# PinataFarms/DAD-3DHeads

Measured on AMD Instinct MI355X. Metric: images/sec (FLAME decode + 445-lmk projection), batch 64 @ 256^2, higher is better.
Workload: dtype f32

## Files before the change

dad-3dheads_amd/csrc/flame_decode_head.hip:

```cpp
#pragma clang fp contract(off)
#include "common.hpp"
#include "flame_math.hpp"
#include "flame_pipe_epilogue.hpp"

#ifndef DAD3D_HEAD_DEPTH
#define DAD3D_HEAD_DEPTH 6
#endif
#ifndef DAD3D_HEAD_R0_AT
#define DAD3D_HEAD_R0_AT 1
#endif

namespace dad3d {

namespace {

using namespace pipe;

constexpr int KG = kPipeKGroups;
constexpr int TV = kPipeTileVerts;
constexpr int kNumBeta = 400;
constexpr int kJawCol = 3 * TV;
constexpr int LD = 424;
constexpr int OS = 76;
constexpr int CS = 24;
constexpr int kRows = 64;
constexpr int kRows1 = 48;
constexpr int kRound = 128;
constexpr int D = DAD3D_HEAD_DEPTH < KG ? DAD3D_HEAD_DEPTH : KG;
static_assert(D >= 6 && DAD3D_HEAD_R0_AT < D, "issue-ahead depth");
struct Lds {
    static constexpr int a_off = 0;
    static constexpr int o_off = a_off + kRows * LD;
    static constexpr int c_off = o_off + kRows * OS;
    static constexpr int y_off = c_off + 2 * kRound * CS;
    static constexpr int v_off = y_off + 4;
    static constexpr int total = v_off + 4 * TV;
    static_assert(total * 4 <= 160 * 1024, "LDS budget of one CU");
};

__device__ __forceinline__ int lds_peek(lds_int* p) { return __hip_atomic_load(p, __ATOMIC_RELAXED, __HIP_MEMORY_SCOPE_WORKGROUP); }
__device__ __forceinline__ void wait_ge(lds_int* p, int target) {
    while (lds_peek(p) < target) __builtin_amdgcn_s_sleep(1);
    asm volatile("" ::: "memory");
}
__device__ __forceinline__ void wait_ge2(lds_int* p, int target, lds_int* q, int target_q) {
    while ((int)(lds_peek(p) < target) | (int)(lds_peek(q) < target_q)) __builtin_amdgcn_s_sleep(1);
    asm volatile("" ::: "memory");
}
__device__ __forceinline__ void arrive(lds_int* p, int lane) {
    asm volatile("s_waitcnt lgkmcnt(0)" ::: "memory");
    if (lane == 0) __hip_atomic_fetch_add(p, 1, __ATOMIC_RELAXED, __HIP_MEMORY_SCOPE_WORKGROUP);
}
__device__ __forceinline__ void phase_barrier() {
    asm volatile("s_waitcnt lgkmcnt(0)\n\ts_barrier" ::: "memory");
}

}

constexpr int kHeadPreloadDwords = 14;
static_assert(4 * kHeadPreloadDwords == 4 * sizeof(void*) + 6 * sizeof(int), "the preloaded range ends with n_lmk");
struct PipeLateArgs {
    const int* lmk_next;
    float *verts3d, *proj, *lmk_xy;
    int32_t* lmk_px;
    float image_size;
};
static_assert((4 * kHeadPreloadDwords) % alignof(PipeLateArgs) == 0, "`late` starts where the preloaded range ends: late_args() reads it there");
template <bool TO2D>
__global__ __launch_bounds__(512, 2) void flame_decode_head_kernel(float* params, const float* bpack, const float4* vtab, unsigned long long* trace_buf, int batch,
                                                                   int n_verts, int n_params, int span_half, unsigned geom, int n_lmk, PipeLateArgs late) {
    PipeArgs a;
    a.params = params, a.bpack = bpack, a.vtab = vtab, a.trace = trace_buf, a.n_params = n_params, a.batch = batch, a.n_half = span_half, a.n_verts = n_verts, a.n_lmk = n_lmk;
    a.flags = pipe_geom_unpack(geom).flags;
    extern __shared__ __attribute__((aligned(16))) float smem[];
    float* abuf = smem + Lds::a_off;
    float* otile = smem + Lds::o_off;
    float* cst = smem + Lds::c_off;
    lds_int* parts = (lds_int*)(smem + Lds::y_off);

    const int tid = threadIdx.x, lane = tid & 63, wave = tid >> 6;
    const int tile = blockIdx.x, v0 = tile * TV;
    const int B = a.batch, P = a.n_params;
    const bool two = B > kRows1;
    unsigned long long* trace = a.trace ? a.trace + ((size_t)tile * 8 + wave) * 32 : nullptr;
    auto stamp = [&](int slot) {
        if (trace && lane == 0) trace[slot] = __builtin_readcyclecounter();
    };
    if (trace && lane == 0) trace[12] = wall_clock64();
    stamp(0);
    if (tid < 4) __hip_atomic_store(parts + tid, 0, __ATOMIC_RELAXED, __HIP_MEMORY_SCOPE_WORKGROUP);
    const unsigned nl = (unsigned)a.n_lmk;
    EpiCtx cx;
    __amdgpu_buffer_rsrc_t rs3, rsp;
    unsigned outs = 0;
    auto late_args = [&]() {
        typedef const __attribute__((address_space(4))) char* kernarg_ptr;
        typedef const __attribute__((address_space(4))) PipeLateArgs* late_ptr;
        kernarg_ptr kp = (kernarg_ptr)__builtin_amdgcn_kernarg_segment_ptr();
        asm volatile("" : "+s"(kp));
        const late_ptr lp = reinterpret_cast<late_ptr>(kp + 4 * kHeadPreloadDwords);
        a.lmk_next = lp->lmk_next, a.verts3d = lp->verts3d, a.proj = lp->proj, a.lmk_xy = lp->lmk_xy, a.lmk_px = lp->lmk_px, a.image_size = lp->image_size;
        rs3 = __builtin_amdgcn_make_buffer_rsrc(reinterpret_cast<char*>(a.verts3d), 0, 0x7fffffff, 0x00020000);
        rsp = __builtin_amdgcn_make_buffer_rsrc(reinterpret_cast<char*>(a.proj), 0, 0x7fffffff, 0x00020000);
        cx.lx = reinterpret_cast<char*>(a.lmk_xy), cx.lp = reinterpret_cast<char*>(a.lmk_px);
        outs = __builtin_amdgcn_readfirstlane((a.verts3d ? 1u : 0u) | (a.proj ? 2u : 0u));
        asm volatile("" : "+s"(outs));
        cx.lmk_next = a.lmk_next;
        cx.image_size = a.image_size;
    };
    cx.zsign = (a.flags & DAD3D_FLIP_Z) ? -1.0f : 1.0f;
    float4* const vt_lds = reinterpret_cast<float4*>(smem + Lds::v_off);
    auto fin4 = [&](int row0, int w) {
        const int fi = lane & 3, fu = lane >> 2, b = row0 + 4 * w + fi;
        const float4* cp = reinterpret_cast<const float4*>(cst + b * CS);
        const float4 c0 = cp[0], c1 = cp[1], c2 = cp[2], c3 = cp[3], c4 = cp[4], c5 = cp[5];
        const float* ot = otile + b * OS;
        const float jx = ot[kJawCol], jy = ot[kJawCol + 1], jz = ot[kJawCol + 2];
        const unsigned vrow = (unsigned)b * (unsigned)a.n_verts + (unsigned)(v0 + fu), bnl = (unsigned)b * nl;
        {
            const float4 t = vt_lds[fu];
            const bool live = b < B && v0 + fu < a.n_verts;
            finish_vertex<TO2D, 0>(cx, rs3, rsp, c0, c1, c2, c3, c4, c5, jx, jy, jz, ot[3 * fu], ot[3 * fu + 1], ot[3 * fu + 2], t.x, t.y, __float_as_int(t.z), __float_as_int(t.w),
                                   live && (outs & 1u), live && (outs & 2u), live && nl > 0 && __float_as_int(t.z) >= 0, vrow, bnl);
        }
        if (fu < TV - 16) {
            const int j = fu + 16;
            const float4 t = vt_lds[j];
            const bool live = b < B && v0 + j < a.n_verts;
            finish_vertex<TO2D, 16>(cx, rs3, rsp, c0, c1, c2, c3, c4, c5, jx, jy, jz, ot[3 * j], ot[3 * j + 1], ot[3 * j + 2], t.x, t.y, __float_as_int(t.z), __float_as_int(t.w),
                                    live && (outs & 1u), live && (outs & 2u), live && nl > 0 && __float_as_int(t.z) >= 0, vrow, bnl);
        }
    };
    auto fin2 = [&](int row0) {
        const int fi = lane & 1, fu = min(lane >> 1, TV - 1), b = row0 + 2 * wave + fi;
        const float4* cp = reinterpret_cast<const float4*>(cst + b * CS);
        const float4 c0 = cp[0], c1 = cp[1], c2 = cp[2], c3 = cp[3], c4 = cp[4], c5 = cp[5];
        const float* ot = otile + b * OS;
        const float jx = ot[kJawCol], jy = ot[kJawCol + 1], jz = ot[kJawCol + 2];
        const unsigned vrow = (unsigned)b * (unsigned)a.n_verts + (unsigned)(v0 + fu), bnl = (unsigned)b * nl;
        const float4 t = vt_lds[fu];
        const bool live = b < B && (lane >> 1) < TV && v0 + fu < a.n_verts;
        finish_vertex<TO2D, 0>(cx, rs3, rsp, c0, c1, c2, c3, c4, c5, jx, jy, jz, ot[3 * fu], ot[3 * fu + 1], ot[3 * fu + 2], t.x, t.y, __float_as_int(t.z), __float_as_int(t.w),
                               live && (outs & 1u), live && (outs & 2u), live && nl > 0 && __float_as_int(t.z) >= 0, vrow, bnl);
    };

    if (wave >= 4) {
        const int fw = wave - 4;
        const int lr = lane >> 5, lc = lane & 31;
        float4 pre[19];
        const float* prow[6];
#pragma unroll
        for (int jj = 0; jj < 6; ++jj) prow[jj] = a.params + (size_t)min(12 * fw + 2 * jj + lr, B - 1) * P + 4 * lc;
        auto load_slab = [&](int sl) {
#pragma unroll
            for (int jj = 0; jj < 6; ++jj) {
                const f4u v = *reinterpret_cast<const f4u*>(prow[jj] + 128 * sl);
                pre[6 * sl + jj] = float4{v.x, v.y, v.z, v.w};
                __builtin_amdgcn_sched_barrier(0);
            }
        };
        auto write_slab = [&](int sl) {
#pragma unroll
            for (int jj = 0; jj < 6; ++jj) *reinterpret_cast<float4*>(abuf + (12 * fw + 2 * jj + lr) * LD + 128 * sl + 4 * lc) = pre[6 * sl + jj];
        };
        load_slab(0);
        const float4 vt_row = a.vtab[min(v0 + min(lane, TV - 1), a.n_verts - 1)];
        stamp(1);
        phase_barrier();
        stamp(6);
        load_slab(1);
        load_slab(2);
        {
            const int r = min(lane >> 2, 11);
            const f4u v = *reinterpret_cast<const f4u*>(a.params + (size_t)min(12 * fw + r, B - 1) * P + 384 + 4 * (lane & 3));
            pre[18] = float4{v.x, v.y, v.z, v.w};
        }
        late_args();
        write_slab(0);
        arrive(parts, lane);
        stamp(7);
        write_slab(1);
        arrive(parts + 1, lane);
        write_slab(2);
        if (lane < 48) *reinterpret_cast<float4*>(abuf + (12 * fw + (lane >> 2)) * LD + 384 + 4 * (lane & 3)) = pre[18];
        arrive(parts + 2, lane);
        if (fw == 3 && lane < TV) vt_lds[lane] = vt_row;
        stamp(2);
        if (two) {
            float4 q[7];
            const float* qrow[2];
#pragma unroll
            for (int jj = 0; jj < 2; ++jj) qrow[jj] = a.params + (size_t)min(kRows1 + 4 * fw + 2 * jj + lr, B - 1) * P + 4 * lc;
#pragma unroll
            for (int sl = 0; sl < 3; ++sl)
#pragma unroll
                for (int jj = 0; jj < 2; ++jj) {
                    const f4u v = *reinterpret_cast<const f4u*>(qrow[jj] + 128 * sl);
                    q[2 * sl + jj] = float4{v.x, v.y, v.z, v.w};
                }
            {
                const f4u v = *reinterpret_cast<const f4u*>(a.params + (size_t)min(kRows1 + 4 * fw + min(lane >> 2, 3), B - 1) * P + 384 + 4 * (lane & 3));
                q[6] = float4{v.x, v.y, v.z, v.w};
            }
            stamp(16);
#pragma unroll
            for (int sl = 0; sl < 3; ++sl)
#pragma unroll
                for (int jj = 0; jj < 2; ++jj) *reinterpret_cast<float4*>(abuf + (kRows1 + 4 * fw + 2 * jj + lr) * LD + 128 * sl + 4 * lc) = q[2 * sl + jj];
            if (lane < 16) *reinterpret_cast<float4*>(abuf + (kRows1 + 4 * fw + (lane >> 2)) * LD + 384 + 4 * (lane & 3)) = q[6];
            stamp(17);
        }
        stamp(18);
        phase_barrier();
        stamp(19);
        if (two) {
            fin4(32, fw);
            stamp(21);
            phase_barrier();
            stamp(23);
            fin2(kRows1);
        } else {
            fin4(0, wave);
            fin2(32);
        }
        stamp(5);
        if (trace && lane == 0) trace[13] = wall_clock64();
        return;
    }

    const float4* bsrc = reinterpret_cast<const float4*>(a.bpack) + ((size_t)tile * KG * 4 + wave) * 64 + lane;
    f4u raw0 = {}, raw1 = {};
    f3u raw2 = {};
    float raw_scale = 0.f;
    {
        const float* prow = a.params + (size_t)min(32 * wave + (lane & 31), B - 1) * P + kNumBeta;
        raw0 = *reinterpret_cast<const f4u*>(prow), raw1 = *reinterpret_cast<const f4u*>(prow + 4), raw2 = *reinterpret_cast<const f3u*>(prow + 8);
        raw_scale = prow[12];
    }
    auto write_round = [&]() {
        const float jaw[3] = {raw0.x, raw0.y, raw0.z};
        const float rot6[6] = {raw0.w, raw1.x, raw1.y, raw1.z, raw1.w, raw2.x};
        float Dm[9], G[9];
        rodrigues_minus_identity_lean(jaw, Dm);
        rot6_to_matrix_lean(rot6, G);
        const float sp1 = raw_scale + 1.0f;
        const float s = sp1 < 1e-8f ? 1e-8f : sp1;
        if (wave < 2 && lane < 32) {
            float4* tail = reinterpret_cast<float4*>(abuf + (32 * wave + lane) * LD + kNumBeta);
            tail[0] = float4{Dm[0], Dm[1], Dm[2], Dm[3]};
            tail[1] = float4{Dm[4], Dm[5], Dm[6], Dm[7]};
            tail[2] = float4{Dm[8], 1.0f, 0.f, 0.f};
            tail[3] = float4{0.f, 0.f, 0.f, 0.f};
        }
        if (lane < 32) {
            float4* c = reinterpret_cast<float4*>(cst + (32 * wave + lane) * CS);
            c[0] = float4{Dm[0], Dm[1], Dm[2], Dm[3]};
            c[1] = float4{Dm[4], Dm[5], Dm[6], Dm[7]};
            c[2] = float4{Dm[8], G[0], G[1], G[2]};
            c[3] = float4{G[3], G[4], G[5], G[6]};
            c[4] = float4{G[7], G[8], s, raw2.y};
            c[5] = float4{raw2.z, 0.f, 0.f, 0.f};
            const int b = 32 * wave + lane;
            if ((a.flags & DAD3D_MUTATE_PARAMS) && tile == 0 && b < B)
                store_tz(a.params + ((unsigned)b * (unsigned)P + (unsigned)(kNumBeta + 11)));
        }
    };
    float4 bq[KG];
    const float* afrag0 = abuf + (lane & 15) * LD + 4 * (lane >> 4);
    float* const ot0 = otile + ((lane >> 4) * 4) * OS + wave * 16 + (lane & 15);

    late_args();
    stamp(6);
    phase_barrier();
    stamp(7);
#pragma unroll
    for (int G = 0; G < D; ++G) {
        bq[G] = bsrc[(size_t)G * 256];
        __builtin_amdgcn_sched_barrier(0);
        if (G == DAD3D_HEAD_R0_AT) {
            write_round();
            if (wave < 2) arrive(parts + 2, lane);
            arrive(parts + 3, lane);
            stamp(4);
            __builtin_amdgcn_sched_barrier(0);
        }
    }
    {
        f32x4 acc[3] = {f32x4{0.f, 0.f, 0.f, 0.f}, f32x4{0.f, 0.f, 0.f, 0.f}, f32x4{0.f, 0.f, 0.f, 0.f}};
        float4 af[3], an[3] = {};
        stamp(16);
        wait_ge(parts, 4);
#pragma unroll
        for (int m = 0; m < 3; ++m) af[m] = *reinterpret_cast<const float4*>(afrag0 + m * 16 * LD);
#pragma unroll
        for (int G = 0; G < KG; ++G) {
            if (G + D < KG) bq[G + D] = bsrc[(size_t)(G + D) * 256];
            if (G + 1 == 8) wait_ge(parts + 1, 4);
            if (G + 1 == 16) wait_ge2(parts + 2, 6, parts + 3, 4);
            if (G + 1 < KG) {
#pragma unroll
                for (int m = 0; m < 3; ++m) an[m] = *reinterpret_cast<const float4*>(afrag0 + m * 16 * LD + 16 * (G + 1));
            }
            __builtin_amdgcn_sched_barrier(0);
            if (G == 0) stamp(8);
#pragma unroll
            for (int s = 0; s < 4; ++s) {
                const float bv = s == 0 ? bq[G].x : s == 1 ? bq[G].y : s == 2 ? bq[G].z : bq[G].w;
#pragma unroll
                for (int m = 0; m < 3; ++m) {
                    const float av = s == 0 ? af[m].x : s == 1 ? af[m].y : s == 2 ? af[m].z : af[m].w;
                    acc[m] = __builtin_amdgcn_mfma_f32_16x16x4f32(av, bv, acc[m], 0, 0, 0);
                }
            }
            __builtin_amdgcn_sched_barrier(0);
#pragma unroll
            for (int m = 0; m < 3; ++m) af[m] = an[m];
        }
        stamp(2);
#pragma unroll
        for (int m = 0; m < 3; ++m)
#pragma unroll
            for (int q = 0; q < 4; ++q) ot0[(m * 16 + q) * OS] = acc[m][q];
        stamp(17);
    }
    if (!two) {
        phase_barrier();
        stamp(18);
        stamp(3);
        fin4(0, wave);
        fin2(32);
        stamp(5);
        if (trace && lane == 0) trace[13] = wall_clock64();
        return;
    }
    const int ei = lane & 7, eu = lane >> 3, li = 8 * wave + ei;
    float4 k0, k1, k2, k3, k4, k5;
    {
        const float4* c = reinterpret_cast<const float4*>(cst + li * CS);
        k0 = c[0], k1 = c[1], k2 = c[2], k3 = c[3], k4 = c[4], k5 = c[5];
    }
    phase_barrier();
    stamp(18);
    float vW[3], vw2[3];
    int lh[3], ln[3];
    bool vl[3];
#pragma unroll
    for (int k = 0; k < 3; ++k) {
        const float4 t = vt_lds[min(eu + 8 * k, TV - 1)];
        vW[k] = t.x, vw2[k] = t.y, lh[k] = __float_as_int(t.z), ln[k] = __float_as_int(t.w);
        vl[k] = eu + 8 * k < TV && v0 + eu + 8 * k < a.n_verts;
    }
    float jx = 0.f, jy = 0.f, jz = 0.f, ex = 0.f, ey = 0.f, ez = 0.f;
    const float* const ot_e = otile + li * OS;
    const unsigned e_vrow = (unsigned)li * (unsigned)a.n_verts + (unsigned)(v0 + eu), e_bnl = (unsigned)li * nl;
    bool live3[3], livep[3], livel[3];
#pragma unroll
    for (int k = 0; k < 3; ++k) live3[k] = vl[k] && (outs & 1u), livep[k] = vl[k] && (outs & 2u), livel[k] = vl[k] && nl > 0 && lh[k] >= 0;
    auto epi_fetch = [&](int k) {
        const int j = eu + 8 * k;
        ex = ot_e[3 * j], ey = ot_e[3 * j + 1], ez = ot_e[3 * j + 2];
    };
    auto epi_finish = [&](int k) {
        if (k == 0) finish_vertex<TO2D, 0>(cx, rs3, rsp, k0, k1, k2, k3, k4, k5, jx, jy, jz, ex, ey, ez, vW[0], vw2[0], lh[0], ln[0], live3[0], livep[0], livel[0], e_vrow, e_bnl);
        if (k == 1) finish_vertex<TO2D, 8>(cx, rs3, rsp, k0, k1, k2, k3, k4, k5, jx, jy, jz, ex, ey, ez, vW[1], vw2[1], lh[1], ln[1], live3[1], livep[1], livel[1], e_vrow, e_bnl);
        if (k == 2) finish_vertex<TO2D, 16>(cx, rs3, rsp, k0, k1, k2, k3, k4, k5, jx, jy, jz, ex, ey, ez, vW[2], vw2[2], lh[2], ln[2], live3[2], livep[2], livel[2], e_vrow, e_bnl);
    };
    {
        f32x4 acc = f32x4{0.f, 0.f, 0.f, 0.f};
        const float* afrag = afrag0 + kRows1 * LD;
        float4 af = *reinterpret_cast<const float4*>(afrag), an = {};
        stamp(20);
#pragma unroll
        for (int G = 0; G < KG; ++G) {
            if (G + 1 < KG) an = *reinterpret_cast<const float4*>(afrag + 16 * (G + 1));
            __builtin_amdgcn_sched_barrier(0);
            acc = __builtin_amdgcn_mfma_f32_16x16x4f32(af.x, bq[G].x, acc, 0, 0, 0);
            acc = __builtin_amdgcn_mfma_f32_16x16x4f32(af.y, bq[G].y, acc, 0, 0, 0);
            acc = __builtin_amdgcn_mfma_f32_16x16x4f32(af.z, bq[G].z, acc, 0, 0, 0);
            acc = __builtin_amdgcn_mfma_f32_16x16x4f32(af.w, bq[G].w, acc, 0, 0, 0);
            __builtin_amdgcn_sched_barrier(0);
            af = an;
            if (G == 0) {
                jx = ot_e[kJawCol], jy = ot_e[kJawCol + 1], jz = ot_e[kJawCol + 2];
                epi_fetch(0);
            }
            if (G == 3) epi_finish(0), epi_fetch(1);
            if (G == 11) epi_finish(1), epi_fetch(2);
            if (G == 19) epi_finish(2);
            __builtin_amdgcn_sched_barrier(0);
        }
#pragma unroll
        for (int q = 0; q < 4; ++q) ot0[(kRows1 + q) * OS] = acc[q];
        stamp(21);
    }
    phase_barrier();
    stamp(22);
    stamp(3);
    fin2(kRows1);
    stamp(5);
    if (trace && lane == 0) trace[13] = wall_clock64();
}

dad3d_status launch_flame_decode_head(const PipeArgs& a, hipStream_t s) {
    static PerDeviceOnce attr_done;
    const int dev = PerDeviceOnce::current();
    const size_t lds = (size_t)Lds::total * sizeof(float);
    DAD3D_REQUIRE(a.batch > kPipeHalf && a.batch <= kRows && a.chunk_half == 0 && (a.verts3d || a.proj),
                  "launch_flame_decode_head: a whole-mesh launch of 33..64 rows with a vertex output, not %d rows", a.batch);
    if (!attr_done.done(dev)) {
        for (const void* k : {reinterpret_cast<const void*>(&flame_decode_head_kernel<true>), reinterpret_cast<const void*>(&flame_decode_head_kernel<false>)})
            DAD3D_HIP_TRY(hipFuncSetAttribute(k, hipFuncAttributeMaxDynamicSharedMemorySize, (int)lds));
        attr_done.set(dev);
    }
    const bool to2d = (a.flags & DAD3D_TO_2D) || !a.proj;
    const unsigned geom = pipe_geom_word(a.flags, 0, 1, 0);
    const PipeLateArgs late{a.lmk_next, a.verts3d, a.proj, a.lmk_xy, a.lmk_px, a.image_size};
    if (to2d)
        hipLaunchKernelGGL((flame_decode_head_kernel<true>), dim3(a.n_tiles), dim3(512), lds, s, a.params, a.bpack, a.vtab, a.trace, a.batch, a.n_verts, a.n_params, a.n_half, geom,
                           a.n_lmk, late);
    else
        hipLaunchKernelGGL((flame_decode_head_kernel<false>), dim3(a.n_tiles), dim3(512), lds, s, a.params, a.bpack, a.vtab, a.trace, a.batch, a.n_verts, a.n_params, a.n_half, geom,
                           a.n_lmk, late);
    DAD3D_HIP_TRY(hipGetLastError());
    return DAD3D_OK;
}

}
```

Measured before the change: 5.769 million.

## Interleave B-fragment requests and LDS loads among MFMAs; move v16 epilogue to stagers

The global B-fragment prefetch is moved to the middle of each k-step, after the second MFMA row. The next A-fragment LDS reads are issued one per MFMA, spread through the first row, so memory instructions interleave with matrix ops instead of clustering before them. Separately, the epilogue work for vertices 16+ in the 48-row tile leaves the MFMA waves and goes to the staging waves through a new fin_v16 pass, which lightens the compute loop. The risks are more sched_barrier constraints, register pressure, and a possible imbalance between wave groups before the phase barrier.

```diff
diff --git a/dad-3dheads_amd/csrc/flame_decode_head.hip b/dad-3dheads_amd/csrc/flame_decode_head.hip
--- a/dad-3dheads_amd/csrc/flame_decode_head.hip
+++ b/dad-3dheads_amd/csrc/flame_decode_head.hip
@@ -10,11 +10,28 @@
 #define DAD3D_HEAD_R0_AT 1
 #endif
 
+#ifndef DAD3D_HEAD_SPREAD
+#define DAD3D_HEAD_SPREAD 1
+#endif
+#ifndef DAD3D_HEAD_SPREAD_REQ_AT
+#define DAD3D_HEAD_SPREAD_REQ_AT 2
+#endif
+#ifndef DAD3D_HEAD_SPREAD_LDS_AT
+#define DAD3D_HEAD_SPREAD_LDS_AT 4
+#endif
+#ifndef DAD3D_HEAD_V16_STAGERS
+#define DAD3D_HEAD_V16_STAGERS 1
+#endif
+
 namespace dad3d {
 
 namespace {
 
 using namespace pipe;
+constexpr bool kSpread = DAD3D_HEAD_SPREAD != 0;
+constexpr int kSpreadReqAt = DAD3D_HEAD_SPREAD_REQ_AT, kSpreadLdsAt = DAD3D_HEAD_SPREAD_LDS_AT;
+constexpr bool kV16Stagers = DAD3D_HEAD_V16_STAGERS != 0;
+static_assert(kSpreadReqAt >= 0 && kSpreadReqAt < 4 && kSpreadLdsAt >= 0 && kSpreadLdsAt <= 4, "rows of a step's MFMAs");
 
 constexpr int KG = kPipeKGroups;
 constexpr int TV = kPipeTileVerts;
@@ -131,6 +148,18 @@
                                     live && (outs & 1u), live && (outs & 2u), live && nl > 0 && __float_as_int(t.z) >= 0, vrow, bnl);
         }
     };
+    auto fin_v16 = [&](int w) {
+        const int fu = (lane >> 3) & 3, j = fu + 16, b = 8 * w + (lane & 7);
+        const float4* cp = reinterpret_cast<const float4*>(cst + b * CS);
+        const float4 c0 = cp[0], c1 = cp[1], c2 = cp[2], c3 = cp[3], c4 = cp[4], c5 = cp[5];
+        const float* ot = otile + b * OS;
+        const float jx = ot[kJawCol], jy = ot[kJawCol + 1], jz = ot[kJawCol + 2];
+        const unsigned vrow = (unsigned)b * (unsigned)a.n_verts + (unsigned)(v0 + fu), bnl = (unsigned)b * nl;
+        const float4 t = vt_lds[j];
+        const bool live = lane < 32 && v0 + j < a.n_verts;
+        finish_vertex<TO2D, 16>(cx, rs3, rsp, c0, c1, c2, c3, c4, c5, jx, jy, jz, ot[3 * j], ot[3 * j + 1], ot[3 * j + 2], t.x, t.y, __float_as_int(t.z), __float_as_int(t.w),
+                                live && (outs & 1u), live && (outs & 2u), live && nl > 0 && __float_as_int(t.z) >= 0, vrow, bnl);
+    };
     auto fin2 = [&](int row0) {
         const int fi = lane & 1, fu = min(lane >> 1, TV - 1), b = row0 + 2 * wave + fi;
         const float4* cp = reinterpret_cast<const float4*>(cst + b * CS);
@@ -216,6 +245,8 @@
         if (two) {
             fin4(32, fw);
             stamp(21);
+            if (kV16Stagers) fin_v16(fw);
+            stamp(9);
             phase_barrier();
             stamp(23);
             fin2(kRows1);
@@ -294,13 +325,19 @@
         for (int m = 0; m < 3; ++m) af[m] = *reinterpret_cast<const float4*>(afrag0 + m * 16 * LD);
 #pragma unroll
         for (int G = 0; G < KG; ++G) {
-            if (G + D < KG) bq[G + D] = bsrc[(size_t)(G + D) * 256];
+            auto request = [&]() {
+                if (G + D < KG) bq[G + D] = bsrc[(size_t)(G + D) * 256];
+            };
+            auto next_a = [&]() {
+                if (G + 1 < KG) {
+#pragma unroll
+                    for (int m = 0; m < 3; ++m) an[m] = *reinterpret_cast<const float4*>(afrag0 + m * 16 * LD + 16 * (G + 1));
+                }
+            };
+            if (!kSpread) request();
             if (G + 1 == 8) wait_ge(parts + 1, 4);
             if (G + 1 == 16) wait_ge2(parts + 2, 6, parts + 3, 4);
-            if (G + 1 < KG) {
-#pragma unroll
-                for (int m = 0; m < 3; ++m) an[m] = *reinterpret_cast<const float4*>(afrag0 + m * 16 * LD + 16 * (G + 1));
-            }
+            if (!kSpread) next_a();
             __builtin_amdgcn_sched_barrier(0);
             if (G == 0) stamp(8);
 #pragma unroll
@@ -310,6 +347,21 @@
                 for (int m = 0; m < 3; ++m) {
                     const float av = s == 0 ? af[m].x : s == 1 ? af[m].y : s == 2 ? af[m].z : af[m].w;
                     acc[m] = __builtin_amdgcn_mfma_f32_16x16x4f32(av, bv, acc[m], 0, 0, 0);
+                    if (kSpread && kSpreadLdsAt == 4 && s == 0 && G + 1 < KG) {
+                        __builtin_amdgcn_sched_barrier(0);
+                        an[m] = *reinterpret_cast<const float4*>(afrag0 + m * 16 * LD + 16 * (G + 1));
+                        __builtin_amdgcn_sched_barrier(0);
+                    }
+                }
+                if (kSpread && s == kSpreadReqAt) {
+                    __builtin_amdgcn_sched_barrier(0);
+                    request();
+                    __builtin_amdgcn_sched_barrier(0);
+                }
+                if (kSpread && s == kSpreadLdsAt) {
+                    __builtin_amdgcn_sched_barrier(0);
+                    next_a();
+                    __builtin_amdgcn_sched_barrier(0);
                 }
             }
             __builtin_amdgcn_sched_barrier(0);
@@ -385,8 +437,11 @@
                 epi_fetch(0);
             }
             if (G == 3) epi_finish(0), epi_fetch(1);
-            if (G == 11) epi_finish(1), epi_fetch(2);
-            if (G == 19) epi_finish(2);
+            if (G == 11) {
+                epi_finish(1);
+                if (!kV16Stagers) epi_fetch(2);
+            }
+            if (G == 19 && !kV16Stagers) epi_finish(2);
             __builtin_amdgcn_sched_barrier(0);
         }
 #pragma unroll
```

Result: faster. 5.947 million (median of 6 runs) (+3.1%).
